# ucas-vg/PointTinyBenchmark

Measured on AMD Instinct MI355X. Metric: img/s (640x640) CPR R50-FPN fwd+loss, higher is better.
Workload: dtype fp32

## Files before the change

include/cpr_hip.h:

```cpp
#ifndef CPR_HIP_H
#define CPR_HIP_H
#ifdef __cplusplus
extern "C" {
#endif

#define CPR_ERR_ARG (-1001)
#define CPR_ERR_UNSUPPORTED (-1002)

int cpr_version(void);

#define CPR_CONV_RELU 1
#define CPR_CONV_OUT_BF16 2
#define CPR_CONV_RES_MASK 4
#define CPR_CONV_COLSUM 8
int cpr_conv2d_fwd(const float* in, const float* wgt, float* out, const float* scale, const float* bias,
                   const float* residual, const float* in_a, const float* in_b, float* gn_part, int N, int H, int W,
                   int Cin, int Cout, int KH, int KW, int stride, int pad, int Kpad, int flags, int in_relu,
                   int* variant_out, void* stream);

int cpr_conv2d_dual_fwd(const float* in, const float* wgt, const float* in2, const float* wgt2, float* out,
                        const float* scale, const float* bias, const float* scale2, const float* bias2, int N, int H, int W,
                        int Cin, int Cout, int KH, int KW, int stride, int pad, int Kpad, int H2, int W2, int Cin2,
                        int stride2, int Kpad2, int flags, int* variant_out, void* stream);

int cpr_conv1x1_stream_fwd(const float* in, const float* wgt, float* out, const float* scale, const float* bias,
                           const float* residual, long long M, int Cin, int Cout, int flags, void* stream);

int cpr_conv_wgrad_bf16_workspace_s(int N, int H, int W, int Cin, int Cout, int k, int stride, int dy_bf16, int x_bf16);
int cpr_conv_wgrad_bf16_s(const void* dy, int dy_bf16, const void* x, int x_bf16, float* grad, void* ws, int N, int H, int W, int Cin,
// ... 242 lines not shown
typedef struct cpr_preprocess_job {
    const unsigned char* src;
    long long out_off;
    double scale_x, scale_y;
    int pitch, src_w, src_h, x0, y0, cw, ch, dw, dh, flip, Hp, Wp;
} cpr_preprocess_job;
int cpr_preprocess_jobs_u8(const void* jobs_dev, int n_jobs, const float* mean3, const float* stdinv3, int to_rgb, float* out,
                           long long total_out_pixels, void* stream);
int cpr_scale_clip_flip_boxes(float* boxes, const int* img_of, const int* flip, const int* img_hw, const float* scale4, int n,
                              int clip, void* stream);

#ifdef CPR_BENCH_HOOKS
int cpr_conv_force_tile(int bm, int bn);
int cpr_conv_set_pipeline(int mode);
int cpr_conv_set_stream(int on);
int cpr_conv_set_ablation(int mode);
int cpr_wgrad_set_ablation(int mode);
int cpr_conv_set_extra_lds(int bytes);
int cpr_wino_set_variant(int sched, int ablate);
int cpr_bf16_set_dma(int on);
int cpr_bf16_set_wfrag(int on);
int cpr_wino_set_staging(int var, int tpx);
int cpr_wino32_set_debug(int ablate, int wg_per_cu, int stagger_pct);
int cpr_lsa_phase_clocks(long long* host_out, int reset);
int cpr_bn_set_finalize_only(int on);
#endif

#ifdef __cplusplus
}
#endif
// ... 2 lines not shown
```

pointtinybenchmark_amd/_lib.py:

```python
import ctypes
import os

_HERE = os.path.dirname(os.path.abspath(__file__))
LIB_PATH = os.path.join(_HERE, 'csrc', 'libcprhip.so')

_p = ctypes.c_void_p
_i = ctypes.c_int
_f = ctypes.c_float
_l = ctypes.c_longlong
_d = ctypes.c_double

SIGNATURES = {
    'cpr_version': [],
    'cpr_conv2d_fwd': [_p, _p, _p, _p, _p, _p, _p, _p, _p, _i, _i, _i, _i, _i, _i, _i, _i, _i, _i, _i, _i, _p, _p],
    'cpr_conv2d_dual_fwd': [_p] * 9 + [_i] * 16 + [_p, _p],
    'cpr_conv1x1_stream_fwd': [_p, _p, _p, _p, _p, _p, _l, _i, _i, _i, _p],
    'cpr_conv_wgrad_bf16_workspace_s': [_i] * 9,
    'cpr_conv_wgrad_bf16_s': [_p, _i, _p, _i, _p, _p] + [_i] * 8 + [_p],
    'cpr_wino_pack_weights': [_p, _p, _i, _i, _i, _p],
    'cpr_conv3x3_wino_fwd': [_p, _p, _p, _p, _p, _p, _p, _p, _i, _i, _i, _i, _i, _i, _i, _i, _p],
    'cpr_wino32_pack_weights': [_p, _p, _i, _i, _i, _p],
    'cpr_conv3x3_wino32_slots': [_i, _i],
    'cpr_conv3x3_wino32_fwd': [_p, _p, _p, _p, _p, _p, _p, _p, _i, _i, _i, _i, _i, _i, _i, _i, _p],
    'cpr_conv3x3_wino_wgrad_workspace': [_i, _i, _i, _i, _i],
# ... 94 lines not shown
    'cpr_p2p_out_bf16_wgrad_ws': [_i] * 5,
    'cpr_p2p_out_bf16_wgrad': [_p] * 4 + [_i] + [_p] * 3 + [_i] * 5 + [_p],
    'cpr_p2p_loss_bwd': [_p] * 9 + [_i] * 5 + [_f] * 9 + [_p, _i, _i, _p],
    'cpr_p2p_loss_bwd_levels': [_p] * 7 + [_i] * 5 + [_p] * 6 + [_f] * 9 + [_p, _i, _i, _p],
    'cpr_grad_sumsq': [_p, _l, _p, _p, _i, _p],
    'cpr_sgd_step': [_p, _p, _p, _p, _l, _f, _f, _f, _f, _f, _i, _p],
    'cpr_adam_step': [_p, _p, _p, _p, _p, _l, _d, _d, _d, _d, _d, _f, _f, _f, _f, _i, _p],
}

BENCH_SIGNATURES = {
    'cpr_lsa_phase_clocks': [_p, _i],
    'cpr_wino32_set_debug': [_i, _i, _i],
    'cpr_conv_force_tile': [_i, _i],
    'cpr_conv_set_pipeline': [_i],
    'cpr_conv_set_stream': [_i],
    'cpr_conv_set_ablation': [_i],
    'cpr_wgrad_set_ablation': [_i],
    'cpr_wino_set_variant': [_i, _i],
    'cpr_wino_set_staging': [_i, _i],
    'cpr_conv_set_extra_lds': [_i],
    'cpr_bf16_set_dma': [_i],
    'cpr_bf16_set_wfrag': [_i],
    'cpr_bn_set_finalize_only': [_i],
}
BENCH_LIB_PATH = os.path.join(_HERE, 'csrc', 'libcprhip_bench.so')

_lib = None


class CprHipError(RuntimeError):
# ... 37 lines not shown
```

pointtinybenchmark_amd/csrc/common.h:

```cpp
#pragma once
#include <hip/hip_runtime.h>
#include <stdint.h>

#define CPR_OK 0
#define CPR_ERR_ARG (-1001)
#define CPR_ERR_UNSUPPORTED (-1002)

#define CPR_CONV_RELU 1
#define CPR_CONV_OUT_BF16 2
#define CPR_CONV_RES_MASK 4
#define CPR_CONV_COLSUM 8

#define CPR_WINO_IN_B8 1
#define CPR_WINO_OUT_B8 2

#define CPR_CHECK_ARG(cond) \
    do {                    \
        if (!(cond)) return CPR_ERR_ARG; \
    } while (0)

#define CPR_LAUNCH_STATUS()                          \
    do {                                             \
        hipError_t e_ = hipGetLastError();           \
        return e_ == hipSuccess ? CPR_OK : -(int)e_; \
    } while (0)

// ... 70 lines not shown
```

pointtinybenchmark_amd/csrc/conv_mfma.hip:

```cpp
#include <type_traits>
#include "common.h"

struct ConvParams {
    const float* in;
    const float* wgt;
    float* out;
    const float* scale;
    const float* bias;
    const float* residual;
    const float* in_a;
    const float* in_b;
    float* gn_part;
    int N, H, W, Cin, OH, OW, Cout, KH, KW, stride, pad, Kpad, M, relu, in_relu, out_bf16;
    int res_mask;
    int tilesM, tilesN;
    const float* in2;
    const float* wgt2;
    const float* scale2;
    const float* bias2;
    int H2, W2, Cin2, stride2, Kpad2;
};

constexpr int BK = 32;
constexpr int LDSW = 36;

template <int BM, int BN, int MODE, bool XF, int PIPE, int ABL = 0, bool DUAL = false>
__global__ __launch_bounds__(256, 2) void conv_mfma_kernel(ConvParams p) {
    static_assert(!DUAL || (MODE == 0 && !XF && PIPE == 1 && ABL == 0), "the dual-source form exists for the plain pipelined instances");
    constexpr int WM = BM / 2;
    constexpr int WN = BN / 2;
    constexpr int MI = WM / 32;
    constexpr int NI = WN / 32;
    constexpr int AL = BM * 8 / 256;
    constexpr int BL = BN * 8 / 256;
    constexpr int XFMAX = 512;
    __shared__ __attribute__((aligned(16))) float smem[2 * (BM + BN) * LDSW + (XF ? 2 * XFMAX : 0)];
    float* As = smem;
    float* Bs = smem + 2 * BM * LDSW;
    float* ABs = smem + 2 * (BM + BN) * LDSW;

    const int T = p.tilesM * p.tilesN;
    const int per = (T + 7) >> 3;
    const int tile = (blockIdx.x & 7) * per + (blockIdx.x >> 3);
    if (tile >= T) return;
    const int tm = tile / p.tilesN, tn = tile - tm * p.tilesN;
    const int m0 = tm * BM, n0 = tn * BN;

    const int tid = threadIdx.x, lane = tid & 63, wave = tid >> 6;
    const int c4 = tid & 7, r0 = tid >> 3;

    int iy0[AL], ix0[AL], nimg[AL], rowoff[AL];
    bool mok[AL];
    const int ohw = p.OH * p.OW;
    const bool gemm = (p.KH == 1) & (p.KW == 1) & (p.stride == 1) & (p.pad == 0) & (MODE == 0);
#pragma unroll
    for (int j = 0; j < AL; ++j) {
        int m = m0 + r0 + 32 * j;
        mok[j] = m < p.M;
        int mm = mok[j] ? m : 0;
        if (gemm) {
            nimg[j] = 0; iy0[j] = 0; ix0[j] = 0;
            rowoff[j] = mm * p.Cin + c4 * 4;
        } else {
            int n = mm / ohw;
            int rem = mm - n * ohw;
            int oy = rem / p.OW, ox = rem - oy * p.OW;
            nimg[j] = n;
            iy0[j] = oy * p.stride - p.pad;
            ix0[j] = ox * p.stride - p.pad;
            rowoff[j] = ((n * p.H + iy0[j]) * p.W + ix0[j]) * p.Cin + c4 * 4;
        }
    }
    __amdgpu_buffer_rsrc_t rs_in = __builtin_amdgcn_make_buffer_rsrc(
        const_cast<float*>(p.in), 0, (int)((size_t)p.N * p.H * p.W * p.Cin * 4), 0x00020000);
    __amdgpu_buffer_rsrc_t rs_w = __builtin_amdgcn_make_buffer_rsrc(
        const_cast<float*>(p.wgt), 0, (int)((size_t)p.Cout * p.Kpad * 4), 0x00020000);
    int cin_cur = p.Cin;
    bool second = false;
    const float* wrow[BL];
    int woff[BL];
    bool wok[BL];
#pragma unroll
    for (int j = 0; j < BL; ++j) {
        int c = n0 + r0 + 32 * j;
        wok[j] = c < p.Cout;
        wrow[j] = p.wgt + (size_t)(wok[j] ? c : 0) * p.Kpad + c4 * 4;
        woff[j] = wok[j] ? (c * p.Kpad + c4 * 4) * 4 : -1;
    }

    constexpr int NSET = (!XF && BM == 64 && BN == 64) ? 2 : 1;
    f32x4 ra[NSET][AL], rb[NSET][BL], xa, xb;
    unsigned okmask = 0;
    bool any_pad = true;
    int tapoff = 0;
    int kh = 0, kw = 0, c0 = 0;
    constexpr bool xform = XF;
    const float relu_floor = p.in_relu ? 0.f : -INFINITY;
    const int nblk = (m0 < p.M ? m0 : 0) / ohw;
    if (XF) {
        for (int i = tid; i < p.Cin; i += 256) {
            ABs[i] = p.in_a[nblk * p.Cin + i];
            ABs[XFMAX + i] = p.in_b[nblk * p.Cin + i];
// ... 141 lines not shown
        store_tile(Set0{}, 0);
        __syncthreads();
        for (int kt = 0; kt < KT; ++kt) {
            const int buf = kt & 1;
            if (kt + 1 < KT) load_tile(Set0{}, kt + 1);
#pragma unroll
            for (int kk = 0; kk < 4; ++kk) {
                f32x4 fa[MI], fb[NI];
                read_frags(buf, kk, fa, fb);
                mfma_group(fa, fb);
            }
            if (kt + 1 < KT) store_tile(Set0{}, buf ^ 1);
            __syncthreads();
        }
    } else {
      auto kloop = [&](f32x16 (&accX)[MI][NI]) {
        f32x4 fa0[MI], fb0[NI], fa1[MI], fb1[NI];
        load_tile(Set0{}, 0);
        store_tile(Set0{}, 0);
        load_tile(Set1{}, 1);
        if (NSET == 2) load_tile(Set0{}, 2);
        __syncthreads();
        read_frags(0, 0, fa0, fb0);
        constexpr int NM = 4 * MI * NI;
        constexpr int NF = MI + NI;
        constexpr int P1 = NF + AL + BL, P2 = NF + AL + 1 + BL;
        constexpr int PPF = (NF + NM - 1) / NM, PP1 = (P1 + NM - 1) / NM, PP2 = (P2 + NM - 1) / NM;
#define MFMA_SLOT(FA, FB, q)                                                                                  \
    accX[((q) / NI) % MI][(q) % NI] = __builtin_amdgcn_mfma_f32_32x32x2f32(                                 \
        FA[((q) / NI) % MI][(q) / (MI * NI)], FB[(q) % NI][(q) / (MI * NI)], accX[((q) / NI) % MI][(q) % NI], 0, 0, 0)
#define FRAG_PIECE(FA, FB, buf, kk, z)                                                                        \
// ... 57 lines not shown
                    if (z < NF && !(ABL & 2)) FRAG_PIECE(fa0, fb0, buf ^ 1, 0, z);
                __builtin_amdgcn_sched_barrier(0);
            }
        };
        if constexpr (NSET == 2) {
            for (int kt = 0; kt < KT; kt += 2) {
                iteration(Set1{}, kt);
                if (kt + 1 < KT) iteration(Set0{}, kt + 1);
            }
        } else {
            for (int kt = 0; kt < KT; ++kt) iteration(Set0{}, kt);
        }
#undef MFMA_SLOT
#undef FRAG_PIECE
      };
      kloop(acc);
      if constexpr (DUAL) {
        rs_in = __builtin_amdgcn_make_buffer_rsrc(const_cast<float*>(p.in2), 0,
                                                  (int)((size_t)p.N * p.H2 * p.W2 * p.Cin2 * 4), 0x00020000);
        rs_w = __builtin_amdgcn_make_buffer_rsrc(const_cast<float*>(p.wgt2), 0, (int)((size_t)p.Cout * p.Kpad2 * 4), 0x00020000);
        okcur = 0;
#pragma unroll
        for (int j = 0; j < AL; ++j) {
            const int mm = mok[j] ? m0 + r0 + 32 * j : 0;
            const int n = mm / ohw;
            const int rem = mm - n * ohw;
            const int oy = rem / p.OW, ox = rem - oy * p.OW;
            okcur |= (mok[j] ? 1u : 0u) << j;
            voffA[j] = mok[j] ? (((n * p.H2 + oy * p.stride2) * p.W2 + ox * p.stride2) * p.Cin2 + c4 * 4) * 4 : -1;
        }
#pragma unroll
        for (int j = 0; j < BL; ++j) woff[j] = wok[j] ? ((n0 + r0 + 32 * j) * p.Kpad2 + c4 * 4) * 4 : -1;
        cin_cur = p.Cin2; second = true;
        kh = 0; kw = 0; c0 = 0;
        KT = p.Kpad2 / BK; kt_last = KT - 1;
        kloop(acc2);
      }
    }

    const int half = lane >> 5;
    const unsigned row_bytes = (unsigned)p.Cout * 4u;
    const __amdgpu_buffer_rsrc_t rs_out = __builtin_amdgcn_make_buffer_rsrc(
        p.out, 0, (int)((size_t)p.M * p.Cout * 4), 0x00020000);
    const __amdgpu_buffer_rsrc_t rs_res = __builtin_amdgcn_make_buffer_rsrc(
        const_cast<float*>(p.residual ? p.residual : p.out), 0, (int)((size_t)p.M * p.Cout * 4), 0x00020000);
#pragma unroll
    for (int j = 0; j < NI; ++j) {
        const int c = n0 + wn * WN + j * 32 + (lane & 31);
        const bool cok = c < p.Cout;
        const int cc = cok ? c : p.Cout - 1;
        const float sc = p.scale ? p.scale[cc] : 1.f;
// ... 59 lines not shown
                float s = smem[tid * 2] + smem[(BN + tid) * 2];
                float q = smem[tid * 2 + 1] + smem[(BN + tid) * 2 + 1];
                p.gn_part[((size_t)tm * p.Cout + c) * 2 + 0] = s;
                p.gn_part[((size_t)tm * p.Cout + c) * 2 + 1] = q;
            }
        }
    }
}

#ifdef CPR_BENCH_HOOKS
static int force_tile_bm = 0, force_tile_bn = 0;
static int conv_stream_on = 1;
static int conv_pipeline = 1;
static int conv_ablate = 0;
static int conv_extra_lds = 0;

extern "C" int cpr_conv_set_extra_lds(int bytes) {
    CPR_CHECK_ARG(bytes >= 0 && bytes <= 65536);
    conv_extra_lds = bytes;
    return CPR_OK;
}
extern "C" int cpr_conv_set_ablation(int mode) {
    CPR_CHECK_ARG(mode >= 0 && mode <= 16);
    conv_ablate = mode;
    return CPR_OK;
}
extern "C" int cpr_conv_set_stream(int on) {
    CPR_CHECK_ARG(on == 0 || on == 1);
    conv_stream_on = on;
    return CPR_OK;
}
extern "C" int cpr_conv_set_pipeline(int mode) {
    CPR_CHECK_ARG(mode == 0 || mode == 1);
    conv_pipeline = mode;
    return CPR_OK;
}
extern "C" int cpr_conv_force_tile(int bm, int bn) {
    CPR_CHECK_ARG((bm == 0 || bm == 64 || bm == 128) && (bn == 0 || bn == 64 || bn == 128));
    force_tile_bm = bm;
    force_tile_bn = bn;
    return CPR_OK;
}
#else
constexpr int force_tile_bm = 0, force_tile_bn = 0, conv_pipeline = 1, conv_ablate = 0, conv_extra_lds = 0, conv_stream_on = 1;
#endif

int conv1x1_stream_launch(const float* in, const float* wgt, float* out, const float* scale, const float* bias,
                          const float* residual, long long M, int Cin, int Cout, int relu, int res_mask, int min_tiles,
                          hipStream_t stream);
constexpr int STREAM_MIN_TILES = 1024;

static int conv2d_fwd_launch(const float* in, const float* wgt, float* out, const float* scale, const float* bias,
                             const float* residual, const float* in_a, const float* in_b, float* gn_part, int N,
                             int H, int W, int Cin, int Cout, int KH, int KW, int stride, int pad, int Kpad,
                             int flags, int in_relu, int bm_fix, int* variant_out, hipStream_t stream) {
    CPR_CHECK_ARG(in && wgt && out);
    CPR_CHECK_ARG(N > 0 && H > 0 && W > 0 && Cin > 0 && Cout > 0 && KH > 0 && KW > 0 && stride > 0 && pad >= 0);
    CPR_CHECK_ARG(Kpad % BK == 0);
    ConvParams p;
    p.in = in; p.wgt = wgt; p.out = out; p.scale = scale; p.bias = bias; p.residual = residual;
    p.in_a = in_a; p.in_b = in_b; p.gn_part = gn_part;
    p.N = N; p.H = H; p.W = W; p.Cin = Cin; p.Cout = Cout; p.KH = KH; p.KW = KW; p.stride = stride; p.pad = pad;
    CPR_CHECK_ARG((flags & ~15) == 0);
    p.Kpad = Kpad; p.relu = flags & CPR_CONV_RELU; p.in_relu = in_relu; p.out_bf16 = (flags & CPR_CONV_OUT_BF16) ? 1 : 0;
    p.res_mask = (flags & CPR_CONV_RES_MASK) ? 1 : 0;
    p.in2 = nullptr; p.wgt2 = nullptr; p.scale2 = nullptr; p.bias2 = nullptr; p.H2 = p.W2 = p.Cin2 = p.stride2 = p.Kpad2 = 0;
    const bool colsum_mode = (flags & CPR_CONV_COLSUM) != 0;
    if (p.res_mask) CPR_CHECK_ARG(residual != nullptr);
    p.OH = (H + 2 * pad - KH) / stride + 1;
    p.OW = (W + 2 * pad - KW) / stride + 1;
    CPR_CHECK_ARG(p.OH > 0 && p.OW > 0);
    long long M = (long long)N * p.OH * p.OW;
    if ((long long)N * H * W * Cin * 4 >= (1ll << 31) || (long long)Cout * Kpad * 4 >= (1ll << 31) || M >= (1ll << 31) ||
        M * Cout * 4 >= (1ll << 31))
        return CPR_ERR_UNSUPPORTED;
    p.M = (int)M;
    const bool mode1 = (Cin == 4);
    if (!mode1) {
// ... 14 lines not shown
    }
    int bm = 128, bn = (Cout <= 64) ? 64 : 128;
    if ((!gn_part || colsum_mode) && !in_a && !mode1) {
        const long long t128 = (long long)((p.M + 127) / 128) * ((Cout + 127) / 128);
        const int kt = Kpad / BK;
        if (!(kt >= 16 && t128 >= 4096 && Cout > 64)) { bm = 64; bn = 64; }
    }
    if (force_tile_bm > 0 && (!gn_part || colsum_mode) && !in_a && !mode1) { bm = force_tile_bm; }
    if (bm_fix > 0) bm = bm_fix;
    if (force_tile_bn > 0 && Cout > 64 && !mode1) { bn = force_tile_bn; }
    if (variant_out) *variant_out = bm * 1000000 + bn * 1000 + (mode1 ? 100 : 0) + (in_a ? 10 : 0) + conv_pipeline;
    p.tilesM = (p.M + bm - 1) / bm;
    p.tilesN = (Cout + bn - 1) / bn;
    const int T = p.tilesM * p.tilesN;
    const int grid = ((T + 7) / 8) * 8;
#ifdef CPR_BENCH_HOOKS
#define LAUNCH(BM_, BN_, MODE_, XF_)                                                                               \
    do {                                                                                                           \
        if (conv_pipeline == 0)                                                                                    \
            hipLaunchKernelGGL((conv_mfma_kernel<BM_, BN_, MODE_, XF_, 0>), dim3(grid), dim3(256), conv_extra_lds, stream, p); \
        else                                                                                                       \
            hipLaunchKernelGGL((conv_mfma_kernel<BM_, BN_, MODE_, XF_, 1>), dim3(grid), dim3(256), conv_extra_lds, stream, p); \
    } while (0)
#else
#define LAUNCH(BM_, BN_, MODE_, XF_) \
    hipLaunchKernelGGL((conv_mfma_kernel<BM_, BN_, MODE_, XF_, 1>), dim3(grid), dim3(256), 0, stream, p)
#endif
#ifdef CPR_BENCH_HOOKS
    if (conv_ablate && !mode1 && !in_a && bm == 128 && bn == 128) {
        switch (conv_ablate) {
            case 1: hipLaunchKernelGGL((conv_mfma_kernel<128, 128, 0, false, 1, 1>), dim3(grid), dim3(256), 0, stream, p); break;
            case 2: hipLaunchKernelGGL((conv_mfma_kernel<128, 128, 0, false, 1, 2>), dim3(grid), dim3(256), 0, stream, p); break;
            case 3: hipLaunchKernelGGL((conv_mfma_kernel<128, 128, 0, false, 1, 3>), dim3(grid), dim3(256), 0, stream, p); break;
            case 4: hipLaunchKernelGGL((conv_mfma_kernel<128, 128, 0, false, 1, 4>), dim3(grid), dim3(256), 0, stream, p); break;
            case 8: hipLaunchKernelGGL((conv_mfma_kernel<128, 128, 0, false, 1, 8>), dim3(grid), dim3(256), 0, stream, p); break;
            case 16: hipLaunchKernelGGL((conv_mfma_kernel<128, 128, 0, false, 1, 16>), dim3(grid), dim3(256), 0, stream, p); break;
            default: hipLaunchKernelGGL((conv_mfma_kernel<128, 128, 0, false, 1, 7>), dim3(grid), dim3(256), 0, stream, p); break;
        }
    } else
#endif
    if (mode1) {
        if (bn == 64) LAUNCH(128, 64, 1, false); else LAUNCH(128, 128, 1, false);
    } else if (in_a) {
        if (bn == 64) LAUNCH(128, 64, 0, true); else LAUNCH(128, 128, 0, true);
    } else if (bm == 128) {
        if (bn == 64) LAUNCH(128, 64, 0, false); else LAUNCH(128, 128, 0, false);
    } else {
        if (bn == 64) LAUNCH(64, 64, 0, false); else LAUNCH(64, 128, 0, false);
    }
#undef LAUNCH
    CPR_LAUNCH_STATUS();
}

extern "C" int cpr_conv2d_fwd(const float* in, const float* wgt, float* out, const float* scale, const float* bias,
                              const float* residual, const float* in_a, const float* in_b, float* gn_part, int N,
                              int H, int W, int Cin, int Cout, int KH, int KW, int stride, int pad, int Kpad,
                              int flags, int in_relu, int* variant_out, hipStream_t stream) {
    CPR_CHECK_ARG(N > 0 && H > 0 && W > 0 && Cin > 0 && Cout > 0 && KH > 0 && KW > 0 && stride > 0 && pad >= 0);
    const int OH = (H + 2 * pad - KH) / stride + 1, OW = (W + 2 * pad - KW) / stride + 1;
    CPR_CHECK_ARG(OH > 0 && OW > 0);
    const long long in_img = (long long)H * W * Cin * 4, out_img = (long long)OH * OW * Cout * ((flags & CPR_CONV_OUT_BF16) ? 2 : 4);
    const long long res_img = (long long)OH * OW * Cout * 4;
    int align = 1;
    if (flags & CPR_CONV_COLSUM) { const long long r = (long long)OH * OW; align = 1; while ((r * align) % 128 != 0) align *= 2; }
    const int per = cpr_images_per_launch(N, cpr_max2(cpr_max2(in_img, out_img), residual ? res_img : 0), align);
// ... 32 lines not shown
    p.H2 = H2; p.W2 = W2; p.Cin2 = Cin2; p.stride2 = stride2; p.Kpad2 = Kpad2;
    p.tilesM = p.tilesN = 0;
    const long long M = (long long)N * p.OH * p.OW;
    if ((long long)N * H * W * Cin * 4 >= (1ll << 31) || (long long)N * H2 * W2 * Cin2 * 4 >= (1ll << 31) ||
        (long long)Cout * Kpad * 4 >= (1ll << 31) || (long long)Cout * Kpad2 * 4 >= (1ll << 31) || M * Cout * 4 >= (1ll << 31))
        return CPR_ERR_UNSUPPORTED;
    p.M = (int)M;
    int bm = 64, bn = 64;
    const long long t128 = (long long)((p.M + 127) / 128) * ((Cout + 127) / 128);
    if ((Kpad + Kpad2) / BK >= 16 && t128 >= 4096 && Cout > 64) { bm = 128; bn = 128; }
    if (force_tile_bm > 0) { bm = bn = force_tile_bm; }
    if (variant_out) *variant_out = bm * 1000000 + bn * 1000 + 2;
    p.tilesM = (p.M + bm - 1) / bm;
    p.tilesN = (Cout + bn - 1) / bn;
    const int grid = ((p.tilesM * p.tilesN + 7) / 8) * 8;
    if (bm == 64) hipLaunchKernelGGL((conv_mfma_kernel<64, 64, 0, false, 1, 0, true>), dim3(grid), dim3(256), 0, stream, p);
    else hipLaunchKernelGGL((conv_mfma_kernel<128, 128, 0, false, 1, 0, true>), dim3(grid), dim3(256), 0, stream, p);
    CPR_LAUNCH_STATUS();
}

extern "C" int cpr_conv2d_dual_fwd(const float* in, const float* wgt, const float* in2, const float* wgt2, float* out,
                                   const float* scale, const float* bias, const float* scale2, const float* bias2, int N,
                                   int H, int W, int Cin, int Cout, int KH, int KW, int stride, int pad, int Kpad, int H2,
                                   int W2, int Cin2, int stride2, int Kpad2, int flags, int* variant_out, hipStream_t stream) {
    CPR_CHECK_ARG(in && wgt && in2 && wgt2 && out);
    CPR_CHECK_ARG(N > 0 && H > 0 && W > 0 && Cin > 0 && Cout > 0 && KH > 0 && KW > 0 && stride > 0 && pad >= 0);
    CPR_CHECK_ARG(H2 > 0 && W2 > 0 && Cin2 > 0 && stride2 > 0 && (flags & ~CPR_CONV_RELU) == 0);
    CPR_CHECK_ARG(Cin % BK == 0 && Kpad == KH * KW * Cin && Cin2 % BK == 0 && Kpad2 == Cin2);
    const int OH = (H + 2 * pad - KH) / stride + 1, OW = (W + 2 * pad - KW) / stride + 1;
    CPR_CHECK_ARG(OH > 0 && OW > 0 && OH == (H2 - 1) / stride2 + 1 && OW == (W2 - 1) / stride2 + 1);
    const long long img = cpr_max2(cpr_max2((long long)H * W * Cin, (long long)H2 * W2 * Cin2), (long long)OH * OW * Cout) * 4;
    const int per = cpr_images_per_launch(N, img);
    if (per <= 0) return CPR_ERR_UNSUPPORTED;
    for (int n0 = 0; n0 < N; n0 += per) {
        const int n = N - n0 < per ? N - n0 : per;
        const int rc = conv2d_dual_launch(in + (size_t)n0 * H * W * Cin, wgt, in2 + (size_t)n0 * H2 * W2 * Cin2, wgt2,
                                          out + (size_t)n0 * OH * OW * Cout, scale, bias, scale2, bias2, n, H, W, Cin, Cout,
                                          KH, KW, stride, pad, Kpad, H2, W2, Cin2, stride2, Kpad2, flags,
                                          n0 == 0 ? variant_out : nullptr, stream);
        if (rc != CPR_OK) return rc;
    }
    return CPR_OK;
// ... 2 lines not shown
```

pointtinybenchmark_amd/ops.py:

```python
import collections
import ctypes
import math

import torch

from . import _lib


def _ptr(t):
    return ctypes.c_void_p(t.data_ptr()) if t is not None else None


def _stream():
    return ctypes.c_void_p(torch.cuda.current_stream().cuda_stream)


def _check(t, dtype=torch.float32):
    if not t.is_cuda:
        raise _lib.CprHipError('HIP op called with a CPU tensor: the product path has no CPU fallback')
    ok = t.dtype in dtype if isinstance(dtype, tuple) else t.dtype == dtype
    assert ok and t.is_contiguous(), (t.dtype, t.stride())
    return t


# ... 120 lines not shown
        self.Cout, self.Cin, self.KH, self.KW, self.Kpad = Cin, cols_p, KH, KW, Kpad
        self.stride, self.padding = 1, (KH - 1 - padding if pad_override is None else pad_override)
        src = weight.detach()
        if src.dtype != torch.float32 or not src.is_contiguous():
            src = src.float().contiguous()
        self.w = torch.empty((Cin, Kpad), device=weight.device, dtype=torch.float32)
        _lib.call('cpr_pack_weights', _ptr(src), _ptr(scale), _ptr(self.w), Cout, Cin, KH, KW, cols_p, Kpad, 1, _stream())
        self._packed()
        return self

    def out_hw(self, H, W):
        return ((H + 2 * self.padding - self.KH) // self.stride + 1,
                (W + 2 * self.padding - self.KW) // self.stride + 1)


CONV_RELU, CONV_OUT_BF16, CONV_RES_MASK, CONV_COLSUM = 1, 2, 4, 8
WFRAG = [True]
TRACE_CONV_VARIANT = [False, None]

WINOGRAD = [True]
WINO_MIN_FILL = 0.6


def record_ready():
    if not torch.cuda.is_available() or torch.cuda.is_current_stream_capturing():
        return None
    ev = torch.cuda.Event()
    ev.record()
    return ev, torch.cuda.current_stream().cuda_stream


# ... 87 lines not shown
    if TRACE_CONV_VARIANT[0]:
        TRACE_CONV_VARIANT[1] = ('wino32' if inst == '32' else 'wino',
                                 (1 if in_b8 else 0) | (2 if out_b8 else 0) | (4 if in_ab is not None else 0))
    return (out, part) if gn_part else out


def gn_apply_b8(x, a=None, b=None, relu=False):
    assert is_b8(x)
    N, C8, H, W, _ = _check(x, ACT).shape
    y = torch.empty((N, H, W, C8 * 8), device=x.device, dtype=torch.float32)
    _lib.call('cpr_gn_apply_b8', _ptr(x), _ptr(a), _ptr(b), _ptr(y), N, H, W, C8 * 8, int(relu), _stream())
    return y


def conv2d(x, pc, scale=None, bias=None, residual=None, relu=False, in_ab=None, in_relu=False, gn_part=False,
           out=None, out_dtype=None, res_mask=False, colsum=False, out_b8=False):
    _check(x, ACT)
    pack_ready(pc)
    if is_b8(x):
        assert residual is None and not (res_mask or colsum) and out_dtype in (None, torch.float32) and \
            wino_eligible(pc, x.shape[2], x.shape[3], x.dtype), 'channel-blocked input needs a Winograd-eligible layer'
        return conv3x3_wino(x, pc, scale, bias, relu, gn_part, out, in_ab, in_relu, out_b8)
    N, H, W, Cin = x.shape
    assert Cin == pc.Cin, (Cin, pc.Cin)
    assert x.dtype == pc.dtype, 'weights were packed for %s, input is %s' % (pc.dtype, x.dtype)
    OH, OW = pc.out_hw(H, W)
    odt = out_dtype or x.dtype
    if residual is None and not (res_mask or colsum) and odt == torch.float32 and wino_eligible(pc, H, W, x.dtype) and \
            (in_ab is None or Cin <= 512):
        return conv3x3_wino(x, pc, scale, bias, relu, gn_part, out, in_ab, in_relu, out_b8)
    assert not out_b8, 'channel-blocked output is produced by the Winograd layers only (check wino_eligible first)'
# ... 18 lines not shown
                      _ptr(part), N, H, W, Cin, pc.Cout, pc.KH, pc.KW, pc.stride, pc.padding, pc.Kpad, 2,
                      int(odt == torch.float32), vref, _stream())
            if variant is not None:
                TRACE_CONV_VARIANT[1] = ('bf16', variant.value)
            return out, TilePartials(part, slots, pc.Cout)
        _lib.call('cpr_conv2d_fwd_bf16', _ptr(x), _ptr(pc.w), _ptr(pc.frag_image()), _ptr(out), _ptr(scale), _ptr(bias), _ptr(residual),
                  _ptr(part), N, H, W, Cin, pc.Cout, pc.KH, pc.KW, pc.stride, pc.padding, pc.Kpad, int(relu),
                  int(odt == torch.float32), vref, _stream())
        if variant is not None:
            TRACE_CONV_VARIANT[1] = ('bf16', variant.value)
        return (out, part) if gn_part else out
    a = b = None
    if in_ab is not None:
        a, b = in_ab
    flags = (CONV_RELU if relu else 0) | (CONV_OUT_BF16 if odt == torch.bfloat16 else 0) | \
        (CONV_RES_MASK if res_mask else 0) | (CONV_COLSUM if colsum else 0)
    _lib.call('cpr_conv2d_fwd', _ptr(x), _ptr(pc.w), _ptr(out), _ptr(scale), _ptr(bias),
              _ptr(residual), _ptr(a), _ptr(b), _ptr(part), N, H, W, Cin, pc.Cout, pc.KH, pc.KW, pc.stride,
              pc.padding, pc.Kpad, flags, int(in_relu), vref, _stream())
    if variant is not None:
        TRACE_CONV_VARIANT[1] = ('fp32', variant.value)
    if colsum:
        bm = variant.value // 1000000
        return out, TilePartials(part, (N * OH * OW + bm - 1) // bm, pc.Cout)
    return (out, part) if gn_part else out


def conv2d_bf16_mask_slots(x_shape, pc, out_dtype=torch.bfloat16, fused_add=False):
    N, H, W, Cin = x_shape
    if fused_add and (not WFRAG[0] or pc.Cout % 256 != 0):
        return 0
# ... 22 lines not shown
    if variant is not None:
        TRACE_CONV_VARIANT[1] = ('bf16', variant.value)
    return out32, out16, TilePartials(part, slots, pc.Cout)


def conv1x1_stream(x, pc, scale=None, bias=None, residual=None, relu=False, res_mask=False):
    N, H, W, Cin = x.shape
    assert pc.KH == 1 and pc.stride == 1 and pc.padding == 0 and pc.Kpad == Cin and x.dtype == torch.float32
    out = torch.empty((N, H, W, pc.Cout), device=x.device, dtype=torch.float32)
    flags = (CONV_RELU if relu else 0) | (CONV_RES_MASK if res_mask else 0)
    _lib.call('cpr_conv1x1_stream_fwd', _ptr(x), _ptr(pc.w), _ptr(out), _ptr(scale), _ptr(bias), _ptr(residual),
              N * H * W, Cin, pc.Cout, flags, _stream())
    return out


def conv2d_dual(x, pc, x2, pc2, scale=None, bias=None, scale2=None, bias2=None, relu=False, out=None):
    _check(x, ACT)
    _check(x2, ACT)
    pack_ready(pc)
    pack_ready(pc2)
    N, H, W, Cin = x.shape
    N2, H2, W2, Cin2 = x2.shape
    assert x.dtype == torch.float32 and x2.dtype == torch.float32 and pc.dtype == torch.float32 and pc2.dtype == torch.float32
    assert N == N2 and Cin == pc.Cin and Cin2 == pc2.Cin and pc.Cout == pc2.Cout and pc2.KH == 1 and pc2.KW == 1 and pc2.padding == 0
    OH, OW = pc.out_hw(H, W)
    assert (OH, OW) == pc2.out_hw(H2, W2), 'the two sources must produce the same output grid'
    if out is None:
        out = torch.empty((N, OH, OW, pc.Cout), device=x.device, dtype=torch.float32)
    variant = ctypes.c_int(0) if TRACE_CONV_VARIANT[0] else None
    _lib.call('cpr_conv2d_dual_fwd', _ptr(x), _ptr(pc.w), _ptr(x2), _ptr(pc2.w), _ptr(out), _ptr(scale), _ptr(bias),
              _ptr(scale2), _ptr(bias2), N, H, W, Cin, pc.Cout, pc.KH, pc.KW, pc.stride, pc.padding, pc.Kpad, H2, W2, Cin2,
              pc2.stride, pc2.Kpad, CONV_RELU if relu else 0, ctypes.byref(variant) if variant is not None else None, _stream())
    if variant is not None:
        TRACE_CONV_VARIANT[1] = ('fp32', variant.value)
    return out


class TilePartials:

    def __init__(self, part, tiles, C):
        self.part, self.tiles, self.C = part, tiles, C

    def record_stream(self, stream):
        self.part.record_stream(stream)

    def reduce(self):
        cs = torch.empty((self.C,), device=self.part.device, dtype=torch.float32)
# ... 1198 lines not shown
```

Before: 903.9.

## Stage conv MFMA tiles via buffer_load LDS DMA with swizzled layout

Adds an alternative K-loop for the fp32 MFMA implicit-GEMM conv that loads A and B tiles straight from global memory into LDS with buffer_load ... lds. This replaces the register load-then-store staging. It uses an XOR-swizzled LDS layout without padding to avoid bank conflicts, and interleaves the DMA issues and fragment reads with the MFMA slots. It is selected by default for 64x64 tiles with K up to 1152 in the plain and dual-source convs, with flags and a bench hook to force either path. The new path relies on inline asm that sets m0 and on hand-placed waitcnts, so it carries correctness and scheduling risk.

```diff
diff --git a/include/cpr_hip.h b/include/cpr_hip.h
--- a/include/cpr_hip.h
+++ b/include/cpr_hip.h
@@ -13,6 +13,8 @@
 #define CPR_CONV_OUT_BF16 2
 #define CPR_CONV_RES_MASK 4
 #define CPR_CONV_COLSUM 8
+#define CPR_CONV_REG_STAGING 16
+#define CPR_CONV_DMA_STAGING 32
 int cpr_conv2d_fwd(const float* in, const float* wgt, float* out, const float* scale, const float* bias,
                    const float* residual, const float* in_a, const float* in_b, float* gn_part, int N, int H, int W,
                    int Cin, int Cout, int KH, int KW, int stride, int pad, int Kpad, int flags, int in_relu,
@@ -285,6 +287,7 @@
 int cpr_conv_force_tile(int bm, int bn);
 int cpr_conv_set_pipeline(int mode);
 int cpr_conv_set_stream(int on);
+int cpr_conv_set_staging(int mode);
 int cpr_conv_set_ablation(int mode);
 int cpr_wgrad_set_ablation(int mode);
 int cpr_conv_set_extra_lds(int bytes);
diff --git a/pointtinybenchmark_amd/_lib.py b/pointtinybenchmark_amd/_lib.py
--- a/pointtinybenchmark_amd/_lib.py
+++ b/pointtinybenchmark_amd/_lib.py
@@ -132,6 +132,7 @@
     'cpr_conv_force_tile': [_i, _i],
     'cpr_conv_set_pipeline': [_i],
     'cpr_conv_set_stream': [_i],
+    'cpr_conv_set_staging': [_i],
     'cpr_conv_set_ablation': [_i],
     'cpr_wgrad_set_ablation': [_i],
     'cpr_wino_set_variant': [_i, _i],
diff --git a/pointtinybenchmark_amd/csrc/common.h b/pointtinybenchmark_amd/csrc/common.h
--- a/pointtinybenchmark_amd/csrc/common.h
+++ b/pointtinybenchmark_amd/csrc/common.h
@@ -10,6 +10,8 @@
 #define CPR_CONV_OUT_BF16 2
 #define CPR_CONV_RES_MASK 4
 #define CPR_CONV_COLSUM 8
+#define CPR_CONV_REG_STAGING 16
+#define CPR_CONV_DMA_STAGING 32
 
 #define CPR_WINO_IN_B8 1
 #define CPR_WINO_OUT_B8 2
diff --git a/pointtinybenchmark_amd/csrc/conv_mfma.hip b/pointtinybenchmark_amd/csrc/conv_mfma.hip
--- a/pointtinybenchmark_amd/csrc/conv_mfma.hip
+++ b/pointtinybenchmark_amd/csrc/conv_mfma.hip
@@ -1,5 +1,7 @@
 #include <type_traits>
 #include "common.h"
+
+typedef int i32x4 __attribute__((ext_vector_type(4)));
 
 struct ConvParams {
     const float* in;
@@ -24,9 +26,10 @@
 constexpr int BK = 32;
 constexpr int LDSW = 36;
 
-template <int BM, int BN, int MODE, bool XF, int PIPE, int ABL = 0, bool DUAL = false>
+template <int BM, int BN, int MODE, bool XF, int PIPE, int ABL = 0, bool DUAL = false, bool DMA = false>
 __global__ __launch_bounds__(256, 2) void conv_mfma_kernel(ConvParams p) {
     static_assert(!DUAL || (MODE == 0 && !XF && PIPE == 1 && ABL == 0), "the dual-source form exists for the plain pipelined instances");
+    static_assert(!DMA || (MODE == 0 && !XF && PIPE == 1 && ABL == 0), "LDS-DMA staging exists for the plain pipelined instances");
     constexpr int WM = BM / 2;
     constexpr int WN = BN / 2;
     constexpr int MI = WM / 32;
@@ -34,9 +37,10 @@
     constexpr int AL = BM * 8 / 256;
     constexpr int BL = BN * 8 / 256;
     constexpr int XFMAX = 512;
-    __shared__ __attribute__((aligned(16))) float smem[2 * (BM + BN) * LDSW + (XF ? 2 * XFMAX : 0)];
+    constexpr int ROWW = DMA ? BK : LDSW;
+    __shared__ __attribute__((aligned(16))) float smem[2 * (BM + BN) * ROWW + (XF ? 2 * XFMAX : 0)];
     float* As = smem;
-    float* Bs = smem + 2 * BM * LDSW;
+    float* Bs = smem + 2 * BM * ROWW;
     float* ABs = smem + 2 * (BM + BN) * LDSW;
 
     const int T = p.tilesM * p.tilesN;
@@ -48,6 +52,7 @@
 
     const int tid = threadIdx.x, lane = tid & 63, wave = tid >> 6;
     const int c4 = tid & 7, r0 = tid >> 3;
+    const int cu = DMA ? (c4 ^ ((r0 >> 1) & 7)) : c4;
 
     int iy0[AL], ix0[AL], nimg[AL], rowoff[AL];
     bool mok[AL];
@@ -60,7 +65,7 @@
         int mm = mok[j] ? m : 0;
         if (gemm) {
             nimg[j] = 0; iy0[j] = 0; ix0[j] = 0;
-            rowoff[j] = mm * p.Cin + c4 * 4;
+            rowoff[j] = mm * p.Cin + cu * 4;
         } else {
             int n = mm / ohw;
             int rem = mm - n * ohw;
@@ -68,7 +73,7 @@
             nimg[j] = n;
             iy0[j] = oy * p.stride - p.pad;
             ix0[j] = ox * p.stride - p.pad;
-            rowoff[j] = ((n * p.H + iy0[j]) * p.W + ix0[j]) * p.Cin + c4 * 4;
+            rowoff[j] = ((n * p.H + iy0[j]) * p.W + ix0[j]) * p.Cin + cu * 4;
         }
     }
     __amdgpu_buffer_rsrc_t rs_in = __builtin_amdgcn_make_buffer_rsrc(
@@ -85,7 +90,7 @@
         int c = n0 + r0 + 32 * j;
         wok[j] = c < p.Cout;
         wrow[j] = p.wgt + (size_t)(wok[j] ? c : 0) * p.Kpad + c4 * 4;
-        woff[j] = wok[j] ? (c * p.Kpad + c4 * 4) * 4 : -1;
+        woff[j] = wok[j] ? (c * p.Kpad + cu * 4) * 4 : -1;
     }
 
     constexpr int NSET = (!XF && BM == 64 && BN == 64) ? 2 : 1;
@@ -257,7 +262,109 @@
             __syncthreads();
         }
     } else {
-      auto kloop = [&](f32x16 (&accX)[MI][NI]) {
+      const int wv = __builtin_amdgcn_readfirstlane(wave);
+      const int lds_a = (int)(unsigned)(size_t)As + wv * 1024, lds_b = (int)(unsigned)(size_t)Bs + wv * 1024;
+      const size_t in_addr = (size_t)p.in, w_addr = (size_t)p.wgt;
+      i32x4 d_in = {(int)(unsigned)in_addr, (int)(unsigned)(in_addr >> 32) & 0xffff, (int)((size_t)p.N * p.H * p.W * p.Cin * 4), 0x00020000};
+      i32x4 d_w = {(int)(unsigned)w_addr, (int)(unsigned)(w_addr >> 32) & 0xffff, (int)((size_t)p.Cout * p.Kpad * 4), 0x00020000};
+      auto dma = [&](const i32x4& rs, int lds_dst, int voff, int soff_) {
+          const int m0v = __builtin_amdgcn_readfirstlane(lds_dst);
+          const int soff = __builtin_amdgcn_readfirstlane(soff_);
+          asm volatile("s_nop 4\n\ts_mov_b32 m0, %0\n\ts_nop 0\n\tbuffer_load_dwordx4 %1, %2, %3 offen offset:0 lds"
+                       :: "s"(m0v), "v"(voff), "s"(rs), "s"(soff) : "memory");
+      };
+      auto dma_piece = [&](int buf, int kt, int z) {
+          if (z < AL) dma(d_in, lds_a + buf * (BM * BK * 4) + z * 4096, voffA[z < AL ? z : 0], c0 * 4);
+          else if (z == AL) load_x_advance();
+          else dma(d_w, lds_b + buf * (BN * BK * 4) + (z - AL - 1) * 4096, woff[z > AL ? z - AL - 1 : 0], kt * (BK * 4));
+      };
+      const int hx = (lane >> 5) ^ ((lane >> 1) & 7);
+      const float* a_swz = As + arow * BK;
+      const float* b_swz = Bs + brow * BK;
+      auto kloop_dma = [&](f32x16 (&accX)[MI][NI]) {
+        constexpr int NM = 4 * MI * NI, NF = MI + NI, ND = AL + 1 + BL;
+        constexpr int PPF = (NF + NM - 1) / NM, PP3 = (NF + ND + NM - 1) / NM;
+        f32x4 fa0[MI], fb0[NI], fa1[MI], fb1[NI];
+#define MFMA_SLOT(FA, FB, q)                                                                                  \
+    accX[((q) / NI) % MI][(q) % NI] = __builtin_amdgcn_mfma_f32_32x32x2f32(                                 \
+        FA[((q) / NI) % MI][(q) / (MI * NI)], FB[(q) % NI][(q) / (MI * NI)], accX[((q) / NI) % MI][(q) % NI], 0, 0, 0)
+#define FRAG_PIECE(FA, FB, buf, kk, z)                                                                        \
+    do {                                                                                                      \
+        if ((z) < MI)                                                                                         \
+            FA[(z) < MI ? (z) : 0] = *reinterpret_cast<const f32x4*>(a_swz + (buf) * BM * BK +                \
+                                                                     ((z) < MI ? (z) : 0) * 32 * BK + (((2 * (kk)) ^ hx) << 2)); \
+        else                                                                                                  \
+            FB[(z) >= MI ? (z) - MI : 0] = *reinterpret_cast<const f32x4*>(                                   \
+                b_swz + (buf) * BN * BK + ((z) >= MI ? (z) - MI : 0) * 32 * BK + (((2 * (kk)) ^ hx) << 2));    \
+    } while (0)
+#pragma unroll
+        for (int z = 0; z < ND; ++z) dma_piece(0, 0, z);
+        if (KT > 1) {
+#pragma unroll
+            for (int z = 0; z < ND; ++z) dma_piece(1, 1, z);
+            asm volatile("s_waitcnt vmcnt(%0)" :: "n"(AL + BL) : "memory");
+        } else {
+            asm volatile("s_waitcnt vmcnt(0)" ::: "memory");
+        }
+        __builtin_amdgcn_s_barrier();
+        asm volatile("" ::: "memory");
+#pragma unroll
+        for (int z = 0; z < NF; ++z) FRAG_PIECE(fa0, fb0, 0, 0, z);
+        auto iteration = [&](auto buf_c, int kt) {
+            const int buf = buf_c;
+            const bool more = kt + 2 < KT;
+#pragma unroll
+            for (int q = 0; q < NM; ++q) {
+                MFMA_SLOT(fa0, fb0, q);
+#pragma unroll
+                for (int z = q * PPF; z < (q + 1) * PPF; ++z)
+                    if (z < NF) FRAG_PIECE(fa1, fb1, buf, 1, z);
+                __builtin_amdgcn_sched_barrier(0);
+            }
+#pragma unroll
+            for (int q = 0; q < NM; ++q) {
+                MFMA_SLOT(fa1, fb1, q);
+#pragma unroll
+                for (int z = q * PPF; z < (q + 1) * PPF; ++z)
+                    if (z < NF) FRAG_PIECE(fa0, fb0, buf, 2, z);
+                __builtin_amdgcn_sched_barrier(0);
+            }
+#pragma unroll
+            for (int q = 0; q < NM; ++q) {
+                MFMA_SLOT(fa0, fb0, q);
+#pragma unroll
+                for (int z = q * PPF; z < (q + 1) * PPF; ++z)
+                    if (z < NF) FRAG_PIECE(fa1, fb1, buf, 3, z);
+                __builtin_amdgcn_sched_barrier(0);
+            }
+            asm volatile("" ::: "memory");
+            asm volatile("s_waitcnt vmcnt(0) lgkmcnt(0)" ::: "memory");
+            __builtin_amdgcn_s_barrier();
+            asm volatile("" ::: "memory");
+            __builtin_amdgcn_sched_barrier(0);
+#pragma unroll
+            for (int q = 0; q < NM; ++q) {
+                MFMA_SLOT(fa1, fb1, q);
+#pragma unroll
+                for (int z = q * PP3; z < (q + 1) * PP3; ++z) {
+                    if (z < NF) FRAG_PIECE(fa0, fb0, buf ^ 1, 0, z);
+                    else if (z < NF + ND) { if (more) dma_piece(buf, kt + 2, z - NF); }
+                }
+                __builtin_amdgcn_sched_barrier(0);
+            }
+        };
+        if constexpr (BM == 64 && BN == 64) {
+            for (int kt = 0; kt < KT; kt += 2) {
+                iteration(std::integral_constant<int, 0>{}, kt);
+                if (kt + 1 < KT) iteration(std::integral_constant<int, 1>{}, kt + 1);
+            }
+        } else {
+            for (int kt = 0; kt < KT; ++kt) iteration(kt & 1, kt);
+        }
+#undef MFMA_SLOT
+#undef FRAG_PIECE
+      };
+      auto kloop_reg = [&](f32x16 (&accX)[MI][NI]) {
         f32x4 fa0[MI], fb0[NI], fa1[MI], fb1[NI];
         load_tile(Set0{}, 0);
         store_tile(Set0{}, 0);
@@ -345,11 +452,14 @@
 #undef MFMA_SLOT
 #undef FRAG_PIECE
       };
-      kloop(acc);
+      if constexpr (DMA) kloop_dma(acc); else kloop_reg(acc);
       if constexpr (DUAL) {
         rs_in = __builtin_amdgcn_make_buffer_rsrc(const_cast<float*>(p.in2), 0,
                                                   (int)((size_t)p.N * p.H2 * p.W2 * p.Cin2 * 4), 0x00020000);
         rs_w = __builtin_amdgcn_make_buffer_rsrc(const_cast<float*>(p.wgt2), 0, (int)((size_t)p.Cout * p.Kpad2 * 4), 0x00020000);
+        const size_t in2_addr = (size_t)p.in2, w2_addr = (size_t)p.wgt2;
+        d_in = i32x4{(int)(unsigned)in2_addr, (int)(unsigned)(in2_addr >> 32) & 0xffff, (int)((size_t)p.N * p.H2 * p.W2 * p.Cin2 * 4), 0x00020000};
+        d_w = i32x4{(int)(unsigned)w2_addr, (int)(unsigned)(w2_addr >> 32) & 0xffff, (int)((size_t)p.Cout * p.Kpad2 * 4), 0x00020000};
         okcur = 0;
 #pragma unroll
         for (int j = 0; j < AL; ++j) {
@@ -358,14 +468,14 @@
             const int rem = mm - n * ohw;
             const int oy = rem / p.OW, ox = rem - oy * p.OW;
             okcur |= (mok[j] ? 1u : 0u) << j;
-            voffA[j] = mok[j] ? (((n * p.H2 + oy * p.stride2) * p.W2 + ox * p.stride2) * p.Cin2 + c4 * 4) * 4 : -1;
-        }
-#pragma unroll
-        for (int j = 0; j < BL; ++j) woff[j] = wok[j] ? ((n0 + r0 + 32 * j) * p.Kpad2 + c4 * 4) * 4 : -1;
+            voffA[j] = mok[j] ? (((n * p.H2 + oy * p.stride2) * p.W2 + ox * p.stride2) * p.Cin2 + cu * 4) * 4 : -1;
+        }
+#pragma unroll
+        for (int j = 0; j < BL; ++j) woff[j] = wok[j] ? ((n0 + r0 + 32 * j) * p.Kpad2 + cu * 4) * 4 : -1;
         cin_cur = p.Cin2; second = true;
         kh = 0; kw = 0; c0 = 0;
         KT = p.Kpad2 / BK; kt_last = KT - 1;
-        kloop(acc2);
+        if constexpr (DMA) kloop_dma(acc2); else kloop_reg(acc2);
       }
     }
 
@@ -455,6 +565,13 @@
 static int conv_pipeline = 1;
 static int conv_ablate = 0;
 static int conv_extra_lds = 0;
+static int conv_staging = -1;
+
+extern "C" int cpr_conv_set_staging(int mode) {
+    CPR_CHECK_ARG(mode >= -1 && mode <= 1);
+    conv_staging = mode;
+    return CPR_OK;
+}
 
 extern "C" int cpr_conv_set_extra_lds(int bytes) {
     CPR_CHECK_ARG(bytes >= 0 && bytes <= 65536);
@@ -484,11 +601,13 @@
 }
 #else
 constexpr int force_tile_bm = 0, force_tile_bn = 0, conv_pipeline = 1, conv_ablate = 0, conv_extra_lds = 0, conv_stream_on = 1;
+constexpr int conv_staging = -1;
 #endif
 
 int conv1x1_stream_launch(const float* in, const float* wgt, float* out, const float* scale, const float* bias,
                           const float* residual, long long M, int Cin, int Cout, int relu, int res_mask, int min_tiles,
                           hipStream_t stream);
+constexpr int DMA_MAX_K = 1152;
 constexpr int STREAM_MIN_TILES = 1024;
 
 static int conv2d_fwd_launch(const float* in, const float* wgt, float* out, const float* scale, const float* bias,
@@ -502,7 +621,7 @@
     p.in = in; p.wgt = wgt; p.out = out; p.scale = scale; p.bias = bias; p.residual = residual;
     p.in_a = in_a; p.in_b = in_b; p.gn_part = gn_part;
     p.N = N; p.H = H; p.W = W; p.Cin = Cin; p.Cout = Cout; p.KH = KH; p.KW = KW; p.stride = stride; p.pad = pad;
-    CPR_CHECK_ARG((flags & ~15) == 0);
+    CPR_CHECK_ARG((flags & ~63) == 0 && (flags & (CPR_CONV_REG_STAGING | CPR_CONV_DMA_STAGING)) != (CPR_CONV_REG_STAGING | CPR_CONV_DMA_STAGING));
     p.Kpad = Kpad; p.relu = flags & CPR_CONV_RELU; p.in_relu = in_relu; p.out_bf16 = (flags & CPR_CONV_OUT_BF16) ? 1 : 0;
     p.res_mask = (flags & CPR_CONV_RES_MASK) ? 1 : 0;
     p.in2 = nullptr; p.wgt2 = nullptr; p.scale2 = nullptr; p.bias2 = nullptr; p.H2 = p.W2 = p.Cin2 = p.stride2 = p.Kpad2 = 0;
@@ -547,6 +666,11 @@
     p.tilesN = (Cout + bn - 1) / bn;
     const int T = p.tilesM * p.tilesN;
     const int grid = ((T + 7) / 8) * 8;
+    const bool can_dma = !mode1 && !in_a && conv_pipeline == 1;
+    if ((flags & CPR_CONV_DMA_STAGING) && !can_dma) return CPR_ERR_UNSUPPORTED;
+    bool dma = can_dma && bm == 64 && bn == 64 && Kpad <= DMA_MAX_K;
+    if (flags & (CPR_CONV_REG_STAGING | CPR_CONV_DMA_STAGING)) dma = (flags & CPR_CONV_DMA_STAGING) != 0;
+    else if (conv_staging >= 0) dma = can_dma && conv_staging == 1;
 #ifdef CPR_BENCH_HOOKS
 #define LAUNCH(BM_, BN_, MODE_, XF_)                                                                               \
     do {                                                                                                           \
@@ -555,9 +679,13 @@
         else                                                                                                       \
             hipLaunchKernelGGL((conv_mfma_kernel<BM_, BN_, MODE_, XF_, 1>), dim3(grid), dim3(256), conv_extra_lds, stream, p); \
     } while (0)
+#define LAUNCH_DMA(BM_, BN_) \
+    hipLaunchKernelGGL((conv_mfma_kernel<BM_, BN_, 0, false, 1, 0, false, true>), dim3(grid), dim3(256), conv_extra_lds, stream, p)
 #else
 #define LAUNCH(BM_, BN_, MODE_, XF_) \
     hipLaunchKernelGGL((conv_mfma_kernel<BM_, BN_, MODE_, XF_, 1>), dim3(grid), dim3(256), 0, stream, p)
+#define LAUNCH_DMA(BM_, BN_) \
+    hipLaunchKernelGGL((conv_mfma_kernel<BM_, BN_, 0, false, 1, 0, false, true>), dim3(grid), dim3(256), 0, stream, p)
 #endif
 #ifdef CPR_BENCH_HOOKS
     if (conv_ablate && !mode1 && !in_a && bm == 128 && bn == 128) {
@@ -576,12 +704,16 @@
         if (bn == 64) LAUNCH(128, 64, 1, false); else LAUNCH(128, 128, 1, false);
     } else if (in_a) {
         if (bn == 64) LAUNCH(128, 64, 0, true); else LAUNCH(128, 128, 0, true);
+    } else if (dma) {
+        if (bm == 128) { if (bn == 64) LAUNCH_DMA(128, 64); else LAUNCH_DMA(128, 128); }
+        else { if (bn == 64) LAUNCH_DMA(64, 64); else LAUNCH_DMA(64, 128); }
     } else if (bm == 128) {
         if (bn == 64) LAUNCH(128, 64, 0, false); else LAUNCH(128, 128, 0, false);
     } else {
         if (bn == 64) LAUNCH(64, 64, 0, false); else LAUNCH(64, 128, 0, false);
     }
 #undef LAUNCH
+#undef LAUNCH_DMA
     CPR_LAUNCH_STATUS();
 }
 
@@ -644,7 +776,13 @@
     p.tilesM = (p.M + bm - 1) / bm;
     p.tilesN = (Cout + bn - 1) / bn;
     const int grid = ((p.tilesM * p.tilesN + 7) / 8) * 8;
-    if (bm == 64) hipLaunchKernelGGL((conv_mfma_kernel<64, 64, 0, false, 1, 0, true>), dim3(grid), dim3(256), 0, stream, p);
+    bool dma = bm == 64 && Kpad <= DMA_MAX_K && Kpad2 <= DMA_MAX_K;
+    if (flags & (CPR_CONV_REG_STAGING | CPR_CONV_DMA_STAGING)) dma = (flags & CPR_CONV_DMA_STAGING) != 0;
+    else if (conv_staging >= 0) dma = conv_staging == 1;
+    if (dma) {
+        if (bm == 64) hipLaunchKernelGGL((conv_mfma_kernel<64, 64, 0, false, 1, 0, true, true>), dim3(grid), dim3(256), 0, stream, p);
+        else hipLaunchKernelGGL((conv_mfma_kernel<128, 128, 0, false, 1, 0, true, true>), dim3(grid), dim3(256), 0, stream, p);
+    } else if (bm == 64) hipLaunchKernelGGL((conv_mfma_kernel<64, 64, 0, false, 1, 0, true>), dim3(grid), dim3(256), 0, stream, p);
     else hipLaunchKernelGGL((conv_mfma_kernel<128, 128, 0, false, 1, 0, true>), dim3(grid), dim3(256), 0, stream, p);
     CPR_LAUNCH_STATUS();
 }
@@ -655,7 +793,8 @@
                                    int W2, int Cin2, int stride2, int Kpad2, int flags, int* variant_out, hipStream_t stream) {
     CPR_CHECK_ARG(in && wgt && in2 && wgt2 && out);
     CPR_CHECK_ARG(N > 0 && H > 0 && W > 0 && Cin > 0 && Cout > 0 && KH > 0 && KW > 0 && stride > 0 && pad >= 0);
-    CPR_CHECK_ARG(H2 > 0 && W2 > 0 && Cin2 > 0 && stride2 > 0 && (flags & ~CPR_CONV_RELU) == 0);
+    CPR_CHECK_ARG(H2 > 0 && W2 > 0 && Cin2 > 0 && stride2 > 0 && (flags & ~(CPR_CONV_RELU | CPR_CONV_REG_STAGING | CPR_CONV_DMA_STAGING)) == 0);
+    CPR_CHECK_ARG((flags & (CPR_CONV_REG_STAGING | CPR_CONV_DMA_STAGING)) != (CPR_CONV_REG_STAGING | CPR_CONV_DMA_STAGING));
     CPR_CHECK_ARG(Cin % BK == 0 && Kpad == KH * KW * Cin && Cin2 % BK == 0 && Kpad2 == Cin2);
     const int OH = (H + 2 * pad - KH) / stride + 1, OW = (W + 2 * pad - KW) / stride + 1;
     CPR_CHECK_ARG(OH > 0 && OW > 0 && OH == (H2 - 1) / stride2 + 1 && OW == (W2 - 1) / stride2 + 1);
diff --git a/pointtinybenchmark_amd/ops.py b/pointtinybenchmark_amd/ops.py
--- a/pointtinybenchmark_amd/ops.py
+++ b/pointtinybenchmark_amd/ops.py
@@ -158,7 +158,8 @@
                 (W + 2 * self.padding - self.KW) // self.stride + 1)
 
 
-CONV_RELU, CONV_OUT_BF16, CONV_RES_MASK, CONV_COLSUM = 1, 2, 4, 8
+CONV_RELU, CONV_OUT_BF16, CONV_RES_MASK, CONV_COLSUM, CONV_REG_STAGING, CONV_DMA_STAGING = 1, 2, 4, 8, 16, 32
+_STAGING_FLAG = {None: 0, 'reg': CONV_REG_STAGING, 'dma': CONV_DMA_STAGING}
 WFRAG = [True]
 TRACE_CONV_VARIANT = [False, None]
 
@@ -276,7 +277,7 @@
 
 
 def conv2d(x, pc, scale=None, bias=None, residual=None, relu=False, in_ab=None, in_relu=False, gn_part=False,
-           out=None, out_dtype=None, res_mask=False, colsum=False, out_b8=False):
+           out=None, out_dtype=None, res_mask=False, colsum=False, out_b8=False, staging=None):
     _check(x, ACT)
     pack_ready(pc)
     if is_b8(x):
@@ -325,7 +326,7 @@
     if in_ab is not None:
         a, b = in_ab
     flags = (CONV_RELU if relu else 0) | (CONV_OUT_BF16 if odt == torch.bfloat16 else 0) | \
-        (CONV_RES_MASK if res_mask else 0) | (CONV_COLSUM if colsum else 0)
+        (CONV_RES_MASK if res_mask else 0) | (CONV_COLSUM if colsum else 0) | _STAGING_FLAG[staging]
     _lib.call('cpr_conv2d_fwd', _ptr(x), _ptr(pc.w), _ptr(out), _ptr(scale), _ptr(bias),
               _ptr(residual), _ptr(a), _ptr(b), _ptr(part), N, H, W, Cin, pc.Cout, pc.KH, pc.KW, pc.stride,
               pc.padding, pc.Kpad, flags, int(in_relu), vref, _stream())
@@ -378,7 +379,7 @@
     return out
 
 
-def conv2d_dual(x, pc, x2, pc2, scale=None, bias=None, scale2=None, bias2=None, relu=False, out=None):
+def conv2d_dual(x, pc, x2, pc2, scale=None, bias=None, scale2=None, bias2=None, relu=False, out=None, staging=None):
     _check(x, ACT)
     _check(x2, ACT)
     pack_ready(pc)
@@ -394,7 +395,8 @@
     variant = ctypes.c_int(0) if TRACE_CONV_VARIANT[0] else None
     _lib.call('cpr_conv2d_dual_fwd', _ptr(x), _ptr(pc.w), _ptr(x2), _ptr(pc2.w), _ptr(out), _ptr(scale), _ptr(bias),
               _ptr(scale2), _ptr(bias2), N, H, W, Cin, pc.Cout, pc.KH, pc.KW, pc.stride, pc.padding, pc.Kpad, H2, W2, Cin2,
-              pc2.stride, pc2.Kpad, CONV_RELU if relu else 0, ctypes.byref(variant) if variant is not None else None, _stream())
+              pc2.stride, pc2.Kpad, (CONV_RELU if relu else 0) | _STAGING_FLAG[staging],
+              ctypes.byref(variant) if variant is not None else None, _stream())
     if variant is not None:
         TRACE_CONV_VARIANT[1] = ('fp32', variant.value)
     return out
```

Measured after the change: 910.9, median of 6. About the same (+0.8%).
